# tspooner/rl_markets

Hardware: NVIDIA H100
Metric: env steps/sec (batched LOBs) (higher is better)
Workload: dtype f64

## Files before the change

### rl_markets_b200/csrc/rlm_agent.cuh

```cuda
#pragma once
#include "rlm_env.cuh"

#define FULL 0xffffffffu
#define HS_EMPTY (-1)

__device__ __noinline__ unsigned long long mt_next(unsigned long long* x, int& p) {
  int k = p; if (k >= 312) k -= 312;
  const unsigned long long UM = 0xFFFFFFFF80000000ull, LM = 0x7FFFFFFFull, A = 0xB5026F5AA96619E9ull;
  int k1 = k + 1; if (k1 == 312) k1 = 0;
  int km = k + 156; if (km >= 312) km -= 312;
  unsigned long long y = (__ldcg(x + k) & UM) | (__ldcg(x + k1) & LM);
  unsigned long long z = __ldcg(x + km) ^ (y >> 1) ^ ((y & 1ull) ? A : 0ull);
  __stcg(x + k, z);
  p = k + 1;
  z ^= (z >> 29) & 0x5555555555555555ull;
  z ^= (z << 17) & 0x71D67FFFEDA60000ull;
  z ^= (z << 37) & 0xFFF7EEE000000000ull;
  z ^= z >> 43;
  return z;
}
__device__ __noinline__ double mt_uniform_real(unsigned long long* x, int& p) {
  double r = __ull2double_rn(mt_next(x, p)) / 18446744073709551616.0;
  if (r >= 1.0) r = 0.99999999999999988897769753748;
  return r * (1.0 - 0.0) + 0.0;
// ... 112 lines not shown
    }
    unsigned long long sum = __ldg(rnd + ((lane + 449 * nf) & 2047));
#pragma unroll
    for (int i = 0; i < NF_MAX; ++i) sum += v[i];
    out.s[g] = null_state ? 0ull : sum;
  }
  return out;
}
template <bool POW2>
__device__ __forceinline__ int ln_tile(const LnSums& h, int k) {
  if (POW2) {
    const unsigned lo = (unsigned)h.s[k / RLM_MAX_ACTIONS] + P.rg[k / RLM_MAX_ACTIONS][k % RLM_MAX_ACTIONS];
    return h.null_state ? 0 : (int)(lo & (unsigned)(P.memory_size - 1));
  }
  return h.null_state ? 0 : mod_m(h.s[k / RLM_MAX_ACTIONS] + P.rg[k / RLM_MAX_ACTIONS][k % RLM_MAX_ACTIONS]);
}

#define VROW 33
__device__ __forceinline__ double seg_sum(double acc, double w, const double* r) {
#pragma unroll 8
  for (int i = 0; i < 32; ++i) acc += w * r[i];
  return acc;
}
struct QGather { double a[RLM_MAX_ACTIONS]; double b[RLM_MAX_ACTIONS]; };

__device__ __forceinline__ bool occ_test(const unsigned* occ, int f) { return (__ldcg(occ + (f >> 5)) >> (f & 31)) & 1u; }
__device__ __forceinline__ bool occ_test_s(const unsigned* occ_s, int f) { return (occ_s[f >> 5] >> (f & 31)) & 1u; }

__device__ __forceinline__ void q_issue(const unsigned* rnd, const double* th_a, const double* th_b, const float* vars, int n,
                                        bool null_state, int g, int lane, unsigned long long* bases, bool reuse, int* idx,
// ... 335 lines not shown
```

### rl_markets_b200/csrc/rlm_api.cu

```cuda
#include <cuda_runtime.h>
#include <math.h>
#include <stdio.h>
#include <string.h>
#include <algorithm>
#include <mutex>
#include <string>
#include <vector>

#include "rlm.h"
#include "rlm_flow_tables.h"
#include "rlm_rndseq.h"
#include "rlm_kernels.h"
#include <limits.h>
#include <stddef.h>
#include <stdlib.h>

static thread_local std::string g_err;
static int fail(int code, const std::string& msg) { g_err = msg; return code; }
int rlm_set_error_(int code, const std::string& msg) { return fail(code, msg); }
#define CK(expr)                                                                                      \
  do {                                                                                                \
    cudaError_t _e = (expr);                                                                          \
    if (_e != cudaSuccess) return fail((_e == cudaErrorNoDevice || _e == cudaErrorInsufficientDriver) ? RLM_ERR_NO_DEVICE : RLM_ERR_CUDA, \
                                       std::string(#expr) + ": " + cudaGetErrorString(_e));          \
// ... 314 lines not shown
    CK(cudaMemsetAsync(h->ptr.tape_lo, 0, (size_t)cfg->n_envs * sizeof(int), h->stream));
  }
  g_params_owner = nullptr;
  int rc = upload_params(h);
  if (rc != RLM_OK) return rc;
  CK(rlm_launch_init(h->ptr, cfg->n_envs, 0, h->stream));
  CK(rlm_launch_seed(h->ptr, cfg->n_envs, cfg->random_seed, h->stream));
  if (cfg->random_init) CK(rlm_launch_random_init(h->ptr, h->n_policies, h->stream));
  h->alpha = cfg->alpha_start;
  h->eps = (double)cfg->eps_init;
  h->tau = (double)cfg->tau_init;
  memset(&h->dyn, 0, sizeof(h->dyn));
#ifdef RLM_TIMING
  if (const char* s = getenv("RLM_DEBUG_FLAGS")) h->dyn.debug_flags = atoi(s);
#endif
  if (const char* s = getenv("RLM_ENV_HASH")) h->dyn.env_hash = atoi(s) != 0;
  if (const char* s = getenv("RLM_ROUND_CAP")) h->dyn.round_cap = std::max(0, atoi(s));
  CK(cudaDeviceGetAttribute(&h->n_sms, cudaDevAttrMultiProcessorCount, cfg->device));
  CK(cudaMalloc(&h->ptr.ready, (size_t)cfg->n_envs * 4));
  CK(cudaMalloc(&h->ptr.hsum, (size_t)cfg->n_envs * 3 * 32 * 8));
  h->ready_cap = RLM_READY_CAP;
  CK(cudaMalloc(&h->ptr.ready_count, (size_t)2 * RLM_LIVE_OFF * 4));
  CK(cudaMemset(h->ptr.ready_count, 0, (size_t)2 * RLM_LIVE_OFF * 4));
  CK(cudaMalloc(&h->ptr.runctl, sizeof(RunCtl)));
  CK(cudaMemset(h->ptr.runctl, 0, sizeof(RunCtl)));
  CK(cudaMallocHost(&h->h_live, RLM_MAX_SUB * 2 * sizeof(int)));
  for (int s = 0; s < RLM_MAX_SUB; ++s)
    for (int i = 0; i < 2; ++i) CK(cudaEventCreateWithFlags(&h->ev_live[s][i], cudaEventDisableTiming));
  if (const char* s = getenv("RLM_ROUND_STREAMS")) { const int v = atoi(s); if (v >= 1 && v <= RLM_MAX_SUB) h->round_streams = v; }
  h->n_sub = 1;
  h->staged = !h->hp.is_double && !cfg->shared_policy && cfg->memory_size * 8 <= 65536 && (cfg->memory_size % 2) == 0;
// ... 41 lines not shown
      h->rounds_auto = false;
    }
    if (!getenv("RLM_ROUND_CAP")) h->dyn.round_cap = 3;
    if (const char* s = getenv("RLM_PDL")) rlm_set_pdl(atoi(s));
    if (const char* s = getenv("RLM_AGENT_VARIANT")) { const int v = atoi(s); h->agent_variant = (v == 1 || v == 3) ? v : 4; }
    if (cfg->memory_size > (1LL << 27)) {
      if (h->agent_variant == 4) h->agent_variant = 3;
      if (h->engine == 3) h->engine = 1;
    }
  }
  if (cfg->source == RLM_SOURCE_TAPE) {
    if (h->engine != 1) return fail(RLM_ERR_UNSUPPORTED, "the tape source runs on the tick-synchronous and round-paced engines (RLM_ENGINE=F|f|p read the stream source only)");
    h->dyn.tape_l2 = 1;
    if (const char* s = getenv("RLM_TAPE_PREFETCH")) h->dyn.tape_l2 = atoi(s) != 0;
  }
  cudaDeviceSetLimit(cudaLimitMaxL2FetchGranularity, 32);
  CK(cudaStreamSynchronize(h->stream));
  return RLM_OK;
}

int rlm_destroy(rlm_handle h) {
  API_LOCK;
  if (!h) return RLM_OK;
  cudaSetDevice(h->cfg.device);
  cudaStreamSynchronize(h->stream);
  cudaFree(h->ptr.env); cudaFree(h->ptr.theta); cudaFree(h->ptr.theta_b); cudaFree(h->ptr.dtheta);
  cudaFree(h->ptr.trace_f); cudaFree(h->ptr.trace_e); cudaFree(h->ptr.mt_pol); cudaFree(h->ptr.mt_agt);
  cudaFree(h->ptr.records); cudaFree(h->ptr.record_count); cudaFree(h->ptr.counters);
  cudaFree(h->d_gather); if (h->h_gather) cudaFreeHost(h->h_gather);
  if (h->copy_stream) { cudaStreamSynchronize(h->copy_stream); cudaStreamDestroy(h->copy_stream); }
  for (int i = 0; i < 2; ++i) {
    cudaFree(h->d_stream[i]);
    if (h->ev_copied[i]) cudaEventDestroy(h->ev_copied[i]);
    if (h->ev_consumed[i]) cudaEventDestroy(h->ev_consumed[i]);
  }
  cudaFree(h->ptr.ready); cudaFree(h->ptr.ready_count); cudaFree(h->ptr.occ); cudaFree(h->ptr.hsum);
  cudaFree(h->ptr.runctl); if (h->h_live) cudaFreeHost(h->h_live);
  cudaFree((void*)h->ptr.tape); cudaFree(h->ptr.tape_cur); cudaFree(h->ptr.tape_lo);
  for (auto& es : h->ev_live) for (auto e : es) if (e) cudaEventDestroy(e);
  cudaFree(h->ptr.q_slots); cudaFree(h->ptr.ag_done); cudaFree(h->d_qctl);
  for (auto e : h->ev) cudaEventDestroy(e);
  for (auto& g : h->graphs) cudaGraphExecDestroy(g.exec);
  if (h->ev_fork) cudaEventDestroy(h->ev_fork);
  for (int s = 0; s < RLM_MAX_SUB; ++s) {
    if (h->sub_stream[s]) { cudaStreamSynchronize(h->sub_stream[s]); cudaStreamDestroy(h->sub_stream[s]); }
    if (h->ev_join[s]) cudaEventDestroy(h->ev_join[s]);
  }
  if (h->own_stream && h->stream) cudaStreamDestroy(h->stream);
  if (g_params_owner == h) g_params_owner = nullptr;
  delete h;
  return RLM_OK;
// ... 609 lines not shown
  return RLM_OK;
}
int rlm_write_theta(rlm_handle h, int32_t policy, int32_t table, const double* in, int64_t n) {
  API_LOCK;
  if (!h || !in) return fail(RLM_ERR_INVALID_ARGUMENT, "null argument");
  if (policy < 0 || policy >= h->n_policies || n < 0 || n > h->cfg.memory_size) return fail(RLM_ERR_INVALID_ARGUMENT, "bad policy index / length");
  double* dst = table == 0 ? h->ptr.theta : h->ptr.theta_b;
  if (!dst) return fail(RLM_ERR_INVALID_ARGUMENT, "no such table");
  CK(cudaSetDevice(h->cfg.device));
  CK(cudaStreamSynchronize(h->stream));
  CK(cudaMemcpy(dst + (size_t)policy * h->cfg.memory_size, in, (size_t)n * 8, cudaMemcpyHostToDevice));
  CK(cudaMemset(h->ptr.occ + (size_t)policy * h->hp.occ_words, 0xFF, (size_t)h->hp.occ_words * 4));
  if (!h->cfg.shared_policy) {
    const int dense = (int)h->cfg.memory_size;
    CK(cudaMemcpy(h->ptr.env + (size_t)policy * h->hp.env_stride + offsetof(EnvHdr, ag) + offsetof(AgentD, n_occ), &dense, 4, cudaMemcpyHostToDevice));
  }
  CK(cudaDeviceSynchronize());
  return RLM_OK;
}

int rlm_copy_theta(rlm_handle dst, rlm_handle src) {
  API_LOCK;
  if (!dst || !src) return fail(RLM_ERR_INVALID_ARGUMENT, "null handle");
  if (dst->cfg.device != src->cfg.device || dst->n_policies != src->n_policies || dst->cfg.memory_size != src->cfg.memory_size ||
      dst->hp.is_double != src->hp.is_double || dst->cfg.shared_policy != src->cfg.shared_policy)
    return fail(RLM_ERR_INVALID_ARGUMENT, "rlm_copy_theta: handles differ in device, policy count, memory_size or table count");
  CK(cudaSetDevice(dst->cfg.device));
  CK(cudaStreamSynchronize(src->stream));
  CK(cudaStreamSynchronize(dst->stream));
  const size_t tbytes = (size_t)src->n_policies * (size_t)src->cfg.memory_size * 8;
  CK(cudaMemcpy(dst->ptr.theta, src->ptr.theta, tbytes, cudaMemcpyDeviceToDevice));
  if (src->ptr.theta_b) CK(cudaMemcpy(dst->ptr.theta_b, src->ptr.theta_b, tbytes, cudaMemcpyDeviceToDevice));
  CK(cudaMemcpy(dst->ptr.occ, src->ptr.occ, (size_t)src->n_policies * (size_t)src->hp.occ_words * 4, cudaMemcpyDeviceToDevice));
  if (!src->cfg.shared_policy)
    CK(cudaMemcpy2D(dst->ptr.env + offsetof(EnvHdr, ag) + offsetof(AgentD, n_occ), dst->hp.env_stride,
                    src->ptr.env + offsetof(EnvHdr, ag) + offsetof(AgentD, n_occ), src->hp.env_stride, 4, src->cfg.n_envs,
                    cudaMemcpyDeviceToDevice));
  CK(cudaDeviceSynchronize());
  return RLM_OK;
}

int rlm_read_records(rlm_handle h, int32_t env, rlm_step_record* out, int32_t cap, int32_t* n_out) {
  API_LOCK;
  if (!h || !out || !n_out) return fail(RLM_ERR_INVALID_ARGUMENT, "null argument");
  if (env < 0 || env >= h->hp.record_envs) return fail(RLM_ERR_INVALID_ARGUMENT, "env is not recorded (cfg.record_envs)");
  CK(cudaSetDevice(h->cfg.device));
  CK(cudaStreamSynchronize(h->stream));
  int cnt = 0;
  CK(cudaMemcpy(&cnt, h->ptr.record_count + env, 4, cudaMemcpyDeviceToHost));
  int n = std::min(std::min(cnt, h->hp.record_cap), cap);
  if (n > 0) CK(cudaMemcpy(out, h->ptr.records + (size_t)env * h->hp.record_cap, (size_t)n * sizeof(rlm_step_record), cudaMemcpyDeviceToHost));
  *n_out = n;
// ... 285 lines not shown
```

### rl_markets_b200/csrc/rlm_kernels.cu

```cuda
#include <cuda_runtime.h>
#include <stdint.h>
#define RLM_TABLE_QUAL static __device__ const
#include "rlm_flow_tables.h"
#include "rlm_rndseq.h"
#include "rlm_agent.cuh"
#include <cstdio>
#include "rlm_kernels.h"
#define RLM_ENVT_CARVEOUT_DEFAULT 30
#define RLM_SMEM_CARVEOUT 88

#define SCR_Q 0
#define SCR_SS (SCR_Q + 8 * 2 * RLM_MAX_ACTIONS)
#define SCR_IDX (SCR_SS + 4 * SS_SLOTS)
#define SCR_VBUF (SCR_IDX + 4 * 3 * RLM_MAX_ACTIONS * 32)
#define AG_BYTES ((sizeof(AgentD) + 15) & ~(size_t)15)
size_t rlm_scratch_bytes(int is_double) {
  return ((size_t)SCR_VBUF + (size_t)(is_double ? 2 : 1) * RLM_MAX_ACTIONS * VROW * 8 + 15) & ~(size_t)15;
}
size_t rlm_agent_smem_bytes(int warps_per_cta, int scratch_bytes) {
  return (size_t)warps_per_cta * (AG_BYTES + (size_t)scratch_bytes);
}

#define PDL_PROLOGUE() do { asm volatile("griddepcontrol.launch_dependents;" ::: "memory"); asm volatile("griddepcontrol.wait;" ::: "memory"); } while (0)
static bool g_use_pdl = false;
// ... 452 lines not shown
  e.pnl_step += (double)e.position * mpm;
  e.momentum_pnl_step += (double)e.position * mpm;
  e.agg_r += get_reward(e);
  e.agg_pnl += e.pnl_step;
  e.agg_mpm += mpm;
  if (!is_terminal(e) && fabs(e.agg_mpm) < 1e-5) return -1;
  e.pnl_step = e.agg_pnl;
  window_push(e, ring, W_PNLUP, fmax(0.0, e.pnl_step), oldv[W_PNLUP]);
  window_push(e, ring, W_PNLDN, fabs(fmin(0.0, e.pnl_step)), oldv[W_PNLDN]);
  e.ep_reward += e.agg_r;
  e.ep_bandh += e.agg_mpm;
#pragma unroll 1
  for (int i = 0; i < P.n_state_vars; ++i) e.ag.to_vars[i] = (float)get_variable(e, ring, P.state_vars[i]);
  e.ag.last_reward = get_reward(e);
  e.ag.kind = 0;
  e.ag.hs_valid = 0;
  return 0;
}

template <int THREADS, bool TAPE>
__global__ void __launch_bounds__(THREADS) rlm_env_kernel(DevPtrs ptr, DynParams D, int tslot, int only_begin) {
  const int b = D.env0 + blockIdx.x * THREADS + threadIdx.x;
  const int lane = threadIdx.x & 31;
  if (!only_begin) KLOG_BEGIN(0);
  int ready = -1;
  unsigned ticked = 0, errs = 0;
  bool starved = false;
  if (b < (D.n_sub > 0 ? D.env0 + D.n_sub : P.n_envs)) {
    EnvHdr* g = (EnvHdr*)(ptr.env + (size_t)b * P.env_stride);
    const int2 tc = (TAPE && !only_begin) ? ptr.tape_cur[b] : make_int2(0, 0);
    const int ph = g->phase;
// ... 51 lines not shown
          ready = env_tick(e, ring, msg, D.backtest);
          if (was != PH_PREOPEN && ready != -2) ticked = 1;
          if (ready == -2) ready = -1;
        }
      }
      if (ready >= 0 && !ag_in) {
        const int kind = e.ag.kind;
        const double rew = e.ag.last_reward;
        float tv[RLM_N_STATE_MAX];
        for (int i = 0; i < RLM_N_STATE_MAX; ++i) tv[i] = (i < P.n_state_vars) ? e.ag.to_vars[i] : 0.0f;
        const int4* src = (const int4*)g;
        int4* dst = (int4*)&e;
        for (int i = HOT16; i < ALL16; ++i) dst[i] = src[i];
        e.ag.kind = kind;
        if (kind == 0) {
          e.ag.last_reward = rew; e.ag.hs_valid = 0;
          for (int i = 0; i < RLM_N_STATE_MAX; ++i) if (i < P.n_state_vars) e.ag.to_vars[i] = tv[i];
        }
        ag_in = true;
      }
      errs = (unsigned)(e.err | e.ag.err);
      {
        int4* dst = (int4*)g;
        const int4* src = (const int4*)&e;
        for (int i = 0; i < HOT16; ++i) dst[i] = src[i];
        if (ag_in) for (int i = HOT16; i < ALL16; ++i) dst[i] = src[i];
      }
    }
  }
  if (D.hold) {
    bool still = false;
// ... 157 lines not shown
    __syncwarp();
    ready = *w.flag;
    if (ready == 0) {
      if (lane == W_PNLUP || lane == W_PNLDN) window_push(e, ring, lane, pushv[lane], oldv[lane]);
      __syncwarp();
      {
        const bool has = lane < P.n_state_vars;
        const int var = has ? P.state_vars[lane] : -1;
        double x0 = 0.0, x1 = 0.0;
        const bool two = has && var_tick_args(e, ring, var, x0, x1);
        int t0 = 0, t1 = 0, lerr = 0, hint = e.tk_band;
        if (two) { t0 = to_ticks(x0, &lerr, &hint); t1 = to_ticks(x1, &lerr, &hint); }
        if (lerr) atomicOr(&e.err, lerr);
        if (has) e.ag.to_vars[lane] = (float)(two ? var_from_ticks(var, t0, t1) : get_variable(e, ring, var));
      }
      if (lane == 31) { e.ag.last_reward = get_reward(e); e.ag.kind = 0; }
      if (D.env_hash && !D.backtest && !P.shared_policy && P.algorithm < RLM_ALGO_R_LEARN) {
        __syncwarp();
        const LnSums h = ln_hash(rlm_rndseq_table, e.ag.to_vars, false, lane);
        unsigned long long* hs = ptr.hsum + (size_t)env * 96;
        hs[lane] = h.s[0]; hs[32 + lane] = h.s[1]; hs[64 + lane] = h.s[2];
        const double* th_a = ptr.theta + (size_t)env * (size_t)P.memory_size;
        const double* th_b = ptr.theta_b ? ptr.theta_b + (size_t)env * (size_t)P.memory_size : nullptr;
#pragma unroll 1
        for (int g = 0; g < 3; ++g) {
#pragma unroll
          for (int a = 0; a < RLM_MAX_ACTIONS; ++a) {
            if (a < P.n_actions) {
              const int f = mod_m(h.s[g] + P.rg[g][a]);
              asm volatile("prefetch.global.L2 [%0];" ::"l"(th_a + f));
              if (th_b) asm volatile("prefetch.global.L2 [%0];" ::"l"(th_b + f));
            }
          }
        }
        if (lane == 0) e.ag.hs_valid = 1;
      }
    } else if (ready == 1 && D.backtest) {
      if (lane < P.n_state_vars) e.ag.to_vars[lane] = (float)get_variable(e, ring, P.state_vars[lane]);
    }
  }
  __syncwarp();
  return ready;
}

template <bool TAPE>
__global__ void __launch_bounds__(ENVW_WARPS * 32) rlm_env_kernel_w(DevPtrs ptr, DynParams D, int tslot, int only_begin) {
  PDL_PROLOGUE();
  extern __shared__ __align__(16) unsigned char smem[];
  const int tid = threadIdx.x, lane = tid & 31, warp = tid >> 5;
  const int env = D.env0 + blockIdx.x * (blockDim.x >> 5) + warp;
  if (!only_begin) KLOG_BEGIN(0);
  if (env >= (D.n_sub > 0 ? D.env0 + D.n_sub : P.n_envs)) return;
  const EnvWarp w = envw_carve(smem + (size_t)warp * envw_warp_bytes());
  EnvHdr& e = *w.e;
  EnvHdr* g = (EnvHdr*)(ptr.env + (size_t)env * P.env_stride);
  double* ring = (double*)((unsigned char*)g + sizeof(EnvHdr));
  if (only_begin && !g->ag.need_begin) return;
// ... 14 lines not shown
      starved = tc.x >= tc.y;
      if (!starved) {
        ready = envw_tick<true>(w, ring, ptr, D, env, tc.x, tc.y, lane, ticked, tape_word);
        if (lane == 0) ptr.tape_cur[env].x = tc.x + 1;
      }
    } else if (D.ctl_stream) {
      const int4 rc4 = __ldg((const int4*)ptr.runctl);
      DevPtrs pt = ptr;
      pt.stream = (const rlm_tick_msg*)__ldg((const unsigned long long*)ptr.runctl + 2);
      ready = envw_tick(w, ring, pt, D, env, rc4.z + tslot, rc4.w, lane, ticked);
    } else {
      ready = envw_tick(w, ring, ptr, D, env, D.stream_off + tslot, D.stream_ticks, lane, ticked);
    }
  }
  __syncwarp();
  envw_stage_out(g, &e, lane);
  if (!only_begin) KLOG_END(0);
  if (lane == 0) {
    if (ready >= 0) ptr.ready[atomicAdd(&ptr.ready_count[tslot], 1)] = env;
    if (D.hold && ready < 0 && e.phase != PH_DONE && !starved) atomicAdd(&ptr.counters[5], 1ull);
    if (ticked) atomicAdd(&ptr.counters[0], 1ull);
    const unsigned errs = (unsigned)(e.err | e.ag.err);
    if (errs) atomicOr(&ptr.counters[4], (unsigned long long)errs);
  }
}

template <bool TAPE>
__global__ void __launch_bounds__(ENVW_WARPS * 32, 4) rlm_env_round_kernel(DevPtrs ptr, DynParams D, int tslot) {
  PDL_PROLOGUE();
  extern __shared__ __align__(16) unsigned char smem[];
  const int tid = threadIdx.x, lane = tid & 31, warp = tid >> 5;
// ... 36 lines not shown
      ++tc.x;
    } else {
      ready = envw_tick(w, ring, pt, D, env, rc.stream_off + pos, rc.stream_ticks, lane, ticked);
    }
    ++pos; ++n_run;
    if (ready >= 0) break;
  }
  if (lane == 0) {
    e.run_id = rc.run_id; e.run_pos = pos;
    if (tape) {
      ptr.tape_cur[env].x = tc.x;
      if (D.tape_l2 && tc.x < tc.y) asm volatile("prefetch.global.L2 [%0];" ::"l"(ptr.tape + tc.x));
    }
  }
  __syncwarp();
  envw_stage_out(g, &e, lane);
  KLOG_END(0);
  if (lane == 0) {
    if (ready >= 0) ptr.ready[atomicAdd(&ptr.ready_count[tslot], 1)] = env;
    if (ready >= 0 || (e.phase != PH_DONE && pos < rc.n_ticks && !starved)) atomicAdd(&live_count[tslot], 1);
    if (ticked) atomicAdd(&ptr.counters[0], (unsigned long long)ticked);
    const unsigned errs = (unsigned)(e.err | e.ag.err);
    if (errs) atomicOr(&ptr.counters[4], (unsigned long long)errs);
  }
}
__global__ void rlm_runctl_kernel(RunCtl* dst, RunCtl v) { *dst = v; }

__device__ __forceinline__ void emit_record(const DevPtrs& ptr, const EnvHdr* g, int env, const AgentD& ag, const double* theta_a,
                                         const float* vars, int lane) {
  const int* tf = ptr.trace_f + (size_t)env * P.trace_cap;
  const float* te = ptr.trace_e + (size_t)env * P.trace_cap;
// ... 1085 lines not shown
```

### rl_markets_b200/csrc/rlm_learn.cuh

```cuda
#pragma once

#ifndef LN_WARPS
#define LN_WARPS 3
#endif
#define LN_MIN_CTAS (15 / LN_WARPS)
#ifdef RLM_TIMING
#define LPH(i) do { if (lane == 0 && tp_idx < 4096) g_phase_clk[tp_idx * 16 + (i)] = clock64(); } while (0)
#else
#define LPH(i) do { } while (0)
#endif
#define LN_VROW 98
#define LN_AG_BYTES 704

__host__ __device__ inline size_t ln_v_bytes(int is_double) { return (size_t)(is_double ? 2 : 1) * RLM_MAX_ACTIONS * LN_VROW * 8; }
#ifndef UT_LOG2
#define UT_LOG2 10
#endif
#define UT_SLOTS (1 << UT_LOG2)
#define UT_MAX_ENTRIES (UT_SLOTS / 2)
__host__ __device__ inline size_t ln_scratch_bytes(int is_double) {
  return (ln_v_bytes(is_double) + TT_SLOTS * 4 + 2 * UT_SLOTS * 4 + 8 * 2 * RLM_MAX_ACTIONS + 48 + 15) & ~(size_t)15;
}
__host__ __device__ inline size_t ln_warp_bytes(int is_double) { return (size_t)LN_AG_BYTES + ln_scratch_bytes(is_double); }
static_assert(sizeof(AgentD) <= LN_AG_BYTES, "agent block outgrew its shared-memory slot");

template <int K0, int N>
__device__ __forceinline__ void ln_gather_issue(const double* __restrict__ th, const LnSums& h, double* v) {
  const int A = P.n_actions;
  if (P.m_pow2) {
#pragma unroll
    for (int k = 0; k < N; ++k) v[k] = (((K0 + k) % RLM_MAX_ACTIONS) < A) ? __ldcg(th + ln_tile<true>(h, K0 + k)) : 0.0;
  } else {
#pragma unroll
    for (int k = 0; k < N; ++k) v[k] = (((K0 + k) % RLM_MAX_ACTIONS) < A) ? __ldcg(th + ln_tile<false>(h, K0 + k)) : 0.0;
  }
}
template <int K0, int N>
__device__ __forceinline__ void ln_gather_store(const double* v, int lane, double* V) {
  const int A = P.n_actions;
#pragma unroll
  for (int k = 0; k < N; ++k)
    if (((K0 + k) % RLM_MAX_ACTIONS) < A) V[((K0 + k) % RLM_MAX_ACTIONS) * LN_VROW + ((K0 + k) / RLM_MAX_ACTIONS) * 32 + lane] = v[k];
}
template <bool DBL, int GB>
__device__ __forceinline__ void ln_gather(const double* __restrict__ th_a, const double* __restrict__ th_b, const LnSums& h, int lane, double* V) {
  static_assert(GB == 27 || GB == 9, "gather batch: everything, or one feature group at a time");
  double v[GB];
  if (GB == 27) {
    ln_gather_issue<0, GB>(th_a, h, v); ln_gather_store<0, GB>(v, lane, V);
    if (DBL) { ln_gather_issue<0, GB>(th_b, h, v); ln_gather_store<0, GB>(v, lane, V + RLM_MAX_ACTIONS * LN_VROW); }
  } else {
// ... 129 lines not shown
    slot = (slot + 1) & (TT_SLOTS - 1);
  }
}

__device__ __forceinline__ void ln_tt_build(int* tt, const AgentD& ag, int lane) {
  int4* t4 = (int4*)tt;
#pragma unroll
  for (int i = 0; i < TT_SLOTS / 4 / 32; ++i) t4[lane + 32 * i] = make_int4(HS_EMPTY, HS_EMPTY, HS_EMPTY, HS_EMPTY);
  __syncwarp();
  if (!ag.null_from) {
    const int b0 = ag.from_base0[lane];
#pragma unroll 1
    for (int a = 0; a < P.n_actions; ++a) ptt_insert(tt, tile0_from_base(b0, a), a);
  }
  __syncwarp();
}

__device__ __forceinline__ int ln_trace_pass(AgentD& e, const int* tt, int* ut, bool track, int* tf, float* te, double* theta, int action,
                                          float rate, double scaled_update, int lane, const LnSums& h, double* Vp) {
  const bool null_from = e.null_from != 0;
  const int b0 = e.from_base0[lane];
  const float tol = 0.01f;
  int w = 0;
  int ins = 0;
#define LN_UT_FLUSH() do { __syncwarp(); ln_patch_local_ool(ut, scaled_update, h.s[0], h.s[1], h.s[2], h.null_state, lane, Vp); __syncwarp(); ut_clear(ut, lane); __syncwarp(); ins = 0; } while (0)
  if (rate != 0.0f) {
    const int n = e.n_traces;
#pragma unroll 1
    for (int base = 0; base < n; base += 32 * TR_AHEAD) {
      int fq[TR_AHEAD];
// ... 133 lines not shown
  const bool dbg_nofence = false, dbg_nopatch = false;
#endif
  const int kind = ag.kind;
  const int al = lane & 15;
  const bool do_main = (stage != 2) && (kind == 0);
  const bool do_pre = (stage == 2) ? (kind == 0) : (kind == 1 || (kind == 0 && stage == 1));
  const int n_evals = (do_pre ? 1 : 0) + (do_main ? 1 : 0);
  LnSums h;
  h.s[0] = h.s[1] = h.s[2] = 0ull; h.null_state = true;
  double q = 0.0;
#pragma unroll 1
  for (int ev = 0; ev < n_evals; ++ev) {
    const bool is_main = do_main && (ev == n_evals - 1);
    const float* vars = (is_main || stage == 2) ? ag.to_vars : ag.from_vars;
    const bool null_state = is_main ? false : ((kind == 1 || stage == 1) ? ag.null_from != 0 : false);
    if (is_main && ag.hs_valid) {
      const unsigned long long* hs = ptr.hsum + (size_t)env * 96;
      h.s[0] = __ldcg(hs + lane); h.s[1] = __ldcg(hs + 32 + lane); h.s[2] = __ldcg(hs + 64 + lane);
      h.null_state = false;
    } else {
      h = ln_hash(rnd, vars, null_state, lane);
    }
    LPH(2);
    if (DBL || GB != 27) {
      if (is_main) ln_tt_build(tt, ag, lane);
      ln_gather<DBL, GB>(theta_a, theta_b, h, lane, V);
    } else {
      double v[3 * RLM_MAX_ACTIONS];
      ln_gather_issue<0, 27>(theta_a, h, v);
      LPH(3);
      if (is_main) ln_tt_build(tt, ag, lane);
      LPH(4);
      ln_gather_store<0, 27>(v, lane, V);
    }
    __syncwarp();
    LPH(5);
    q = ln_sums(V, DBL, lane);
    __syncwarp();
    LPH(6);
// ... 26 lines not shown
      __syncwarp();
      rate = (float)dec[0];
      scaled = dec[1];
      table = (DBL && dec[2] != 0.0) ? 1 : 0;
    }
    __syncwarp();
    LPH(7);
    int* tf = ptr.trace_f + (size_t)env * P.trace_cap;
    float* te = ptr.trace_e + (size_t)env * P.trace_cap;
    double* th = table ? theta_b : theta_a;
    if (stage == 1) th = table ? ptr.dtheta + P.memory_size : ptr.dtheta;
    const bool local_patch = (stage == 0) && !dbg_nopatch;
    if (local_patch) { ut_clear(ut, lane); __syncwarp(); }
    const int nz = ln_trace_pass(ag, tt, ut, local_patch, tf, te, th, ag.cur_action, rate, scaled, lane, h,
                                 V + (table ? RLM_MAX_ACTIONS * LN_VROW : 0));
    if (lane == 0) { ag.n_traces = nz; ag.sum_traces += nz; ag.hs_valid = 0; }
    sum_z += (lane == 0) ? (unsigned long long)nz : 0ull;
    __syncwarp();
    LPH(8);
    if (env < P.record_envs && !dbg_nofence) __threadfence();
    LPH(9);
    if (env < P.record_envs) { if (RESIDENT) emit_record_res(ptr, hdr, env, ag, theta_a, ag.to_vars, lane); else emit_record_ool(ptr, g, env, ag, theta_a, ag.to_vars, lane); }
    if (stage == 0) {
      if (lane < RLM_N_STATE_MAX + 3) { ag.prev_vars[lane] = ag.from_vars[lane]; ag.from_vars[lane] = ag.to_vars[lane]; }
      ag.from_base0[lane] = mod_m(h.s[0]);
      if (lane == 0) { ag.prev_null = ag.null_from; ag.null_from = 0; ag.n_steps++; ag.ep_step++; ag.need_begin = 1; }
      steps_done++;
      LPH(13);
      if (local_patch) ln_patch_local(ut, scaled, h.s[0], h.s[1], h.s[2], h.null_state, lane, V + (table ? RLM_MAX_ACTIONS * LN_VROW : 0));
      LPH(14);
      __syncwarp();
// ... 359 lines not shown
      int4 t1 = make_int4(0, 0, 0, 0);
      if (lane + 32 < N16) t1 = __ldcg(src + lane + 32);
      dst[lane] = t0;
      if (lane + 32 < N16) dst[lane + 32] = t1;
    }
    __syncwarp();
    const int kind = ag.kind;
    const bool main_step = kind == 0;
    if (main_step) {
      const int n_tr = ag.n_traces;
      if (lane * 32 < n_tr) {
        asm volatile("prefetch.global.L2 [%0];" ::"l"(ptr.trace_f + (size_t)env * P.trace_cap + lane * 32));
        asm volatile("prefetch.global.L2 [%0];" ::"l"(ptr.trace_e + (size_t)env * P.trace_cap + lane * 32));
      }
    }
    LnSums h;
    const bool null_state = (kind == 1) && ag.null_from != 0;
    if (main_step && ag.hs_valid) {
      const unsigned long long* hs = ptr.hsum + (size_t)env * 96;
      h.s[0] = __ldcg(hs + lane); h.s[1] = __ldcg(hs + 32 + lane); h.s[2] = __ldcg(hs + 64 + lane);
      h.null_state = false;
    } else {
      h = ln_hash(rnd, main_step ? ag.to_vars : ag.from_vars, null_state, lane);
    }
    if (P.m_pow2) {
#pragma unroll
      for (int k = 0; k < 3 * RLM_MAX_ACTIONS; ++k)
        if ((k % RLM_MAX_ACTIONS) < A) idx_s[(k % RLM_MAX_ACTIONS) * LS_IROW + (k / RLM_MAX_ACTIONS) * 32 + lane] = (unsigned short)ln_tile<true>(h, k);
    } else {
#pragma unroll
      for (int k = 0; k < 3 * RLM_MAX_ACTIONS; ++k)
        if ((k % RLM_MAX_ACTIONS) < A) idx_s[(k % RLM_MAX_ACTIONS) * LS_IROW + (k / RLM_MAX_ACTIONS) * 32 + lane] = (unsigned short)ln_tile<false>(h, k);
    }
    if (main_step) ln_tt_build(tt, ag, lane);
    __syncwarp();
    {
      unsigned done = 0;
      while (!done)
        asm volatile("{ .reg .pred p; mbarrier.try_wait.parity.shared::cta.b64 p, [%1], %2; selp.u32 %0, 1, 0, p; }" : "=r"(done) : "r"(mbar_a), "r"(parity) : "memory");
// ... 68 lines not shown
        if (total > P.trace_cap) {
          if (lane == 0) ag.err |= ERR_TRACE_OVERFLOW;
          add = add && (pos < P.trace_cap);
          total = P.trace_cap;
        }
        if (add) {
          __stcg(tf + pos, f);
          __stcg(te + pos, 1.0f);
          const double nv = tab[f] + scaled * (double)1.0f;
          tab[f] = nv;
          __stcg(theta + f, nv);
        }
        w = total;
      }
      __syncwarp();
      if (lane == 0) { ag.n_traces = w; ag.sum_traces += w; ag.hs_valid = 0; }
      sum_z += (lane == 0) ? (unsigned long long)w : 0ull;
      if (env < P.record_envs) { __threadfence(); emit_record_ool(ptr, g, env, ag, theta, ag.to_vars, lane); }
      if (lane < RLM_N_STATE_MAX + 3) { ag.prev_vars[lane] = ag.from_vars[lane]; ag.from_vars[lane] = ag.to_vars[lane]; }
      ag.from_base0[lane] = mod_m(h.s[0]);
      if (lane == 0) { ag.prev_null = ag.null_from; ag.null_from = 0; ag.n_steps++; ag.ep_step++; ag.need_begin = 1; }
      steps_done++;
      __syncwarp();
      q = ls_sums(tab, idx_s, lane);
      if (lane < A) { ag.q_from[lane] = q; ag.qb_from[lane] = 0.0; }
    }
    __syncwarp();
    {
      int4* dst = (int4*)&g->ag;
      const int4* src = (const int4*)&ag;
      __stcg(dst + lane, src[lane]);
// ... 36 lines not shown
```

### rl_markets_b200/csrc/rlm_types.h

```cpp
#pragma once
#include <stdint.h>
#include "rlm.h"

#define RLM_NWIN 10
enum { W_MID = 0, W_VLT, W_VNUM, W_VDEN, W_SPREAD, W_TP, W_ASKTX, W_BIDTX, W_PNLUP, W_PNLDN };

enum { PH_PREOPEN = 0, PH_WARMUP = 1, PH_RUN = 2, PH_DONE = 3 };

enum {
  ERR_BAD_PRICE = 1,
  ERR_TICK_RANGE = 2,
  ERR_TRACE_OVERFLOW = 4,
  ERR_INVALID_STATE = 8,
  ERR_STREAM_UNDERRUN = 16
};

struct OrderD {
  double price;
  long long size, q_head, q_tail, executed, initial_queue;
  int live;
  int transactions;
};

struct SideD {
// ... 18 lines not shown
  float from_vars[RLM_N_STATE_MAX + 3];
  float to_vars[RLM_N_STATE_MAX + 3];
  int from_base0[32];
  int crand_r[31];
  int crand_f, crand_b;
  int mt_pol_idx, mt_agt_idx;
  int null_from;
  int n_traces, cur_action;
  int need_begin;
  int kind;
  int ep_step, err;
  int n_occ;
  double rho;
  float prev_vars[RLM_N_STATE_MAX + 3];
  int prev_null;
  int hs_valid;
  int pad[2];
};

struct FillD { long long volume; double proxy, value; };

struct EnvHdr {
  SideD side[2];
  long long position;
  double pnl_step, momentum_pnl_step, ask_quote, bid_quote;
  double agg_r, agg_pnl, agg_mpm;
  double tp_val, ewma_up, ewma_dn;
  double ep_reward, ep_pnl, ep_bandh;
  double w_sum[RLM_NWIN], w_mean[RLM_NWIN], w_s[RLM_NWIN];
  long long n_ticks;
  int w_head[RLM_NWIN], w_count[RLM_NWIN];
// ... 47 lines not shown
  VenueD venue;
  rlm_flow_params flow;
};

struct DynParams {
  double alpha, eps, tau;
  int greedy;
  int n_ticks;
  int stream_ticks;
  int stream_off;
  int env0;
  int backtest;
  int n_sub;
  int sub_idx;
  int debug_flags;
  int env_hash;
  int round_cap;
  int ctl_stream;
  int hold;
  int tape_l2;
};

#define RLM_MAX_SUB 8
#define RLM_READY_CAP 256
#define RLM_LIVE_OFF (RLM_MAX_SUB * RLM_READY_CAP)

struct RunCtl { int run_id, n_ticks, stream_off, stream_ticks; const rlm_tick_msg* stream; long long pad; };

struct DevPtrs {
  unsigned char* env;
  double* theta;
  double* theta_b;
  double* dtheta;
  int* trace_f;
  float* trace_e;
  unsigned long long* mt_pol;
  unsigned long long* mt_agt;
  const rlm_tick_msg* stream;
  rlm_step_record* records;
  int* record_count;
  unsigned long long* counters;
  unsigned* occ;
  unsigned long long* hsum;
  int* ready;
  int* ready_count;
  int* q_slots;
  unsigned* q_head;
  unsigned* q_tail;
  unsigned* env_warps_done;
  int* q_done;
  int* ag_done;
  int q_size;
  int pad;
  RunCtl* runctl;
  const rlm_tick_msg* tape;
  int2* tape_cur;
  int* tape_lo;
};
// ... 1 lines not shown
```

Baseline: 12.30 million.

## Pre-gather next-state theta rows in env kernel for async agent copy

Replaces the opt-in env-side hash and L2 prefetch with a default-on pregather. The env warp now computes the tile hash and gathers the theta values for every tiling and action into a per-env global row buffer. The agent kernel then pulls those rows into shared memory with cp.async, overlapping the copy with the trace-table build. This takes the dependent random gathers off the agent's critical path. The cost is extra global writes and reads plus a new per-env buffer, and the rows could go stale if theta changes between the gather and its use.

```diff
diff --git a/rl_markets_b200/csrc/rlm_agent.cuh b/rl_markets_b200/csrc/rlm_agent.cuh
--- a/rl_markets_b200/csrc/rlm_agent.cuh
+++ b/rl_markets_b200/csrc/rlm_agent.cuh
@@ -150,6 +150,18 @@
     return h.null_state ? 0 : (int)(lo & (unsigned)(P.memory_size - 1));
   }
   return h.null_state ? 0 : mod_m(h.s[k / RLM_MAX_ACTIONS] + P.rg[k / RLM_MAX_ACTIONS][k % RLM_MAX_ACTIONS]);
+}
+
+template <int K0, int N>
+__device__ __forceinline__ void ln_gather_issue(const double* __restrict__ th, const LnSums& h, double* v) {
+  const int A = P.n_actions;
+  if (P.m_pow2) {
+#pragma unroll
+    for (int k = 0; k < N; ++k) v[k] = (((K0 + k) % RLM_MAX_ACTIONS) < A) ? __ldcg(th + ln_tile<true>(h, K0 + k)) : 0.0;
+  } else {
+#pragma unroll
+    for (int k = 0; k < N; ++k) v[k] = (((K0 + k) % RLM_MAX_ACTIONS) < A) ? __ldcg(th + ln_tile<false>(h, K0 + k)) : 0.0;
+  }
 }
 
 #define VROW 33
diff --git a/rl_markets_b200/csrc/rlm_api.cu b/rl_markets_b200/csrc/rlm_api.cu
--- a/rl_markets_b200/csrc/rlm_api.cu
+++ b/rl_markets_b200/csrc/rlm_api.cu
@@ -352,7 +352,6 @@
 #ifdef RLM_TIMING
   if (const char* s = getenv("RLM_DEBUG_FLAGS")) h->dyn.debug_flags = atoi(s);
 #endif
-  if (const char* s = getenv("RLM_ENV_HASH")) h->dyn.env_hash = atoi(s) != 0;
   if (const char* s = getenv("RLM_ROUND_CAP")) h->dyn.round_cap = std::max(0, atoi(s));
   CK(cudaDeviceGetAttribute(&h->n_sms, cudaDevAttrMultiProcessorCount, cfg->device));
   CK(cudaMalloc(&h->ptr.ready, (size_t)cfg->n_envs * 4));
@@ -424,6 +423,9 @@
     h->dyn.tape_l2 = 1;
     if (const char* s = getenv("RLM_TAPE_PREFETCH")) h->dyn.tape_l2 = atoi(s) != 0;
   }
+  h->dyn.pregather = !cfg->shared_policy && cfg->algorithm < RLM_ALGO_R_LEARN && h->agent_variant == 4 && !h->staged &&
+                     h->engine == 1 && h->env_variant == 0;
+  if (h->dyn.pregather) CK(cudaMalloc(&h->ptr.vrow, (size_t)cfg->n_envs * (p.is_double ? 2 : 1) * RLM_MAX_ACTIONS * RLM_PG_ROW * 8));
   cudaDeviceSetLimit(cudaLimitMaxL2FetchGranularity, 32);
   CK(cudaStreamSynchronize(h->stream));
   return RLM_OK;
@@ -444,7 +446,7 @@
     if (h->ev_copied[i]) cudaEventDestroy(h->ev_copied[i]);
     if (h->ev_consumed[i]) cudaEventDestroy(h->ev_consumed[i]);
   }
-  cudaFree(h->ptr.ready); cudaFree(h->ptr.ready_count); cudaFree(h->ptr.occ); cudaFree(h->ptr.hsum);
+  cudaFree(h->ptr.ready); cudaFree(h->ptr.ready_count); cudaFree(h->ptr.occ); cudaFree(h->ptr.hsum); cudaFree(h->ptr.vrow);
   cudaFree(h->ptr.runctl); if (h->h_live) cudaFreeHost(h->h_live);
   cudaFree((void*)h->ptr.tape); cudaFree(h->ptr.tape_cur); cudaFree(h->ptr.tape_lo);
   for (auto& es : h->ev_live) for (auto e : es) if (e) cudaEventDestroy(e);
@@ -1084,6 +1086,7 @@
   if (!h->cfg.shared_policy) {
     const int dense = (int)h->cfg.memory_size;
     CK(cudaMemcpy(h->ptr.env + (size_t)policy * h->hp.env_stride + offsetof(EnvHdr, ag) + offsetof(AgentD, n_occ), &dense, 4, cudaMemcpyHostToDevice));
+    CK(cudaMemset(h->ptr.env + (size_t)policy * h->hp.env_stride + offsetof(EnvHdr, ag) + offsetof(AgentD, pg_valid), 0, 4));
   }
   CK(cudaDeviceSynchronize());
   return RLM_OK;
@@ -1106,6 +1109,7 @@
     CK(cudaMemcpy2D(dst->ptr.env + offsetof(EnvHdr, ag) + offsetof(AgentD, n_occ), dst->hp.env_stride,
                     src->ptr.env + offsetof(EnvHdr, ag) + offsetof(AgentD, n_occ), src->hp.env_stride, 4, src->cfg.n_envs,
                     cudaMemcpyDeviceToDevice));
+  CK(cudaMemset2D(dst->ptr.env + offsetof(EnvHdr, ag) + offsetof(AgentD, pg_valid), dst->hp.env_stride, 0, 4, dst->cfg.n_envs));
   CK(cudaDeviceSynchronize());
   return RLM_OK;
 }
diff --git a/rl_markets_b200/csrc/rlm_kernels.cu b/rl_markets_b200/csrc/rlm_kernels.cu
--- a/rl_markets_b200/csrc/rlm_kernels.cu
+++ b/rl_markets_b200/csrc/rlm_kernels.cu
@@ -490,7 +490,7 @@
   for (int i = 0; i < P.n_state_vars; ++i) e.ag.to_vars[i] = (float)get_variable(e, ring, P.state_vars[i]);
   e.ag.last_reward = get_reward(e);
   e.ag.kind = 0;
-  e.ag.hs_valid = 0;
+  e.ag.pg_valid = 0;
   return 0;
 }
 
@@ -572,7 +572,7 @@
         for (int i = HOT16; i < ALL16; ++i) dst[i] = src[i];
         e.ag.kind = kind;
         if (kind == 0) {
-          e.ag.last_reward = rew; e.ag.hs_valid = 0;
+          e.ag.last_reward = rew; e.ag.pg_valid = 0;
           for (int i = 0; i < RLM_N_STATE_MAX; ++i) if (i < P.n_state_vars) e.ag.to_vars[i] = tv[i];
         }
         ag_in = true;
@@ -760,33 +760,42 @@
         if (lerr) atomicOr(&e.err, lerr);
         if (has) e.ag.to_vars[lane] = (float)(two ? var_from_ticks(var, t0, t1) : get_variable(e, ring, var));
       }
-      if (lane == 31) { e.ag.last_reward = get_reward(e); e.ag.kind = 0; }
-      if (D.env_hash && !D.backtest && !P.shared_policy && P.algorithm < RLM_ALGO_R_LEARN) {
-        __syncwarp();
-        const LnSums h = ln_hash(rlm_rndseq_table, e.ag.to_vars, false, lane);
-        unsigned long long* hs = ptr.hsum + (size_t)env * 96;
-        hs[lane] = h.s[0]; hs[32 + lane] = h.s[1]; hs[64 + lane] = h.s[2];
-        const double* th_a = ptr.theta + (size_t)env * (size_t)P.memory_size;
-        const double* th_b = ptr.theta_b ? ptr.theta_b + (size_t)env * (size_t)P.memory_size : nullptr;
-#pragma unroll 1
-        for (int g = 0; g < 3; ++g) {
-#pragma unroll
-          for (int a = 0; a < RLM_MAX_ACTIONS; ++a) {
-            if (a < P.n_actions) {
-              const int f = mod_m(h.s[g] + P.rg[g][a]);
-              asm volatile("prefetch.global.L2 [%0];" ::"l"(th_a + f));
-              if (th_b) asm volatile("prefetch.global.L2 [%0];" ::"l"(th_b + f));
-            }
-          }
-        }
-        if (lane == 0) e.ag.hs_valid = 1;
-      }
+      const bool pg = D.pregather && !D.backtest;
+      if (lane == 31) { e.ag.last_reward = get_reward(e); e.ag.kind = 0; e.ag.pg_valid = pg ? 1 : 0; }
     } else if (ready == 1 && D.backtest) {
       if (lane < P.n_state_vars) e.ag.to_vars[lane] = (float)get_variable(e, ring, P.state_vars[lane]);
     }
   }
   __syncwarp();
   return ready;
+}
+
+__device__ __forceinline__ void pg_store(const double* v, double* vr) {
+#pragma unroll
+  for (int a = 0; a < RLM_MAX_ACTIONS; ++a)
+    if (a < P.n_actions) __stcg(vr + a * RLM_PG_ROW, v[a]);
+}
+template <int K0>
+__device__ __forceinline__ void pg_group(const double* th, const LnSums& h, double* vr) {
+  double v[RLM_MAX_ACTIONS];
+  ln_gather_issue<K0, RLM_MAX_ACTIONS>(th, h, v);
+  pg_store(v, vr + (K0 / RLM_MAX_ACTIONS) * 32);
+}
+__device__ __forceinline__ double* pg_gather(const DevPtrs& ptr, int env, const float* to_vars, int lane, double* v) {
+  const LnSums h = ln_hash(rlm_rndseq_table, to_vars, false, lane);
+  unsigned long long* hs = ptr.hsum + (size_t)env * 96;
+  hs[lane] = h.s[0]; hs[32 + lane] = h.s[1]; hs[64 + lane] = h.s[2];
+  const size_t tab = (size_t)RLM_MAX_ACTIONS * RLM_PG_ROW;
+  double* vr = ptr.vrow + (size_t)env * (P.is_double ? 2 : 1) * tab + lane;
+  const double* th = ptr.theta + (size_t)env * (size_t)P.memory_size;
+  if (P.is_double) {
+    pg_group<0>(th, h, vr); pg_group<9>(th, h, vr); pg_group<18>(th, h, vr);
+    th = ptr.theta_b + (size_t)env * (size_t)P.memory_size;
+    vr += tab;
+  }
+  pg_group<0>(th, h, vr); pg_group<9>(th, h, vr);
+  ln_gather_issue<18, RLM_MAX_ACTIONS>(th, h, v);
+  return vr + 64;
 }
 
 template <bool TAPE>
@@ -831,7 +840,11 @@
     }
   }
   __syncwarp();
+  const bool pg = ready == 0 && D.pregather && !D.backtest;
+  double pv[RLM_MAX_ACTIONS];
+  double* pvr = pg ? pg_gather(ptr, env, e.ag.to_vars, lane, pv) : nullptr;
   envw_stage_out(g, &e, lane);
+  if (pg) pg_store(pv, pvr);
   if (!only_begin) KLOG_END(0);
   if (lane == 0) {
     if (ready >= 0) ptr.ready[atomicAdd(&ptr.ready_count[tslot], 1)] = env;
@@ -898,7 +911,11 @@
     }
   }
   __syncwarp();
+  const bool pg = ready == 0 && D.pregather && !D.backtest;
+  double pv[RLM_MAX_ACTIONS];
+  double* pvr = pg ? pg_gather(ptr, env, e.ag.to_vars, lane, pv) : nullptr;
   envw_stage_out(g, &e, lane);
+  if (pg) pg_store(pv, pvr);
   KLOG_END(0);
   if (lane == 0) {
     if (ready >= 0) ptr.ready[atomicAdd(&ptr.ready_count[tslot], 1)] = env;
diff --git a/rl_markets_b200/csrc/rlm_learn.cuh b/rl_markets_b200/csrc/rlm_learn.cuh
--- a/rl_markets_b200/csrc/rlm_learn.cuh
+++ b/rl_markets_b200/csrc/rlm_learn.cuh
@@ -24,17 +24,6 @@
 __host__ __device__ inline size_t ln_warp_bytes(int is_double) { return (size_t)LN_AG_BYTES + ln_scratch_bytes(is_double); }
 static_assert(sizeof(AgentD) <= LN_AG_BYTES, "agent block outgrew its shared-memory slot");
 
-template <int K0, int N>
-__device__ __forceinline__ void ln_gather_issue(const double* __restrict__ th, const LnSums& h, double* v) {
-  const int A = P.n_actions;
-  if (P.m_pow2) {
-#pragma unroll
-    for (int k = 0; k < N; ++k) v[k] = (((K0 + k) % RLM_MAX_ACTIONS) < A) ? __ldcg(th + ln_tile<true>(h, K0 + k)) : 0.0;
-  } else {
-#pragma unroll
-    for (int k = 0; k < N; ++k) v[k] = (((K0 + k) % RLM_MAX_ACTIONS) < A) ? __ldcg(th + ln_tile<false>(h, K0 + k)) : 0.0;
-  }
-}
 template <int K0, int N>
 __device__ __forceinline__ void ln_gather_store(const double* v, int lane, double* V) {
   const int A = P.n_actions;
@@ -194,6 +183,29 @@
     for (int a = 0; a < P.n_actions; ++a) ptt_insert(tt, tile0_from_base(b0, a), a);
   }
   __syncwarp();
+}
+
+template <bool DBL>
+__device__ __forceinline__ void ln_rows_issue(const double* __restrict__ vr, int lane, double* V) {
+  constexpr int ROW = RLM_PG_ROW / 2;
+  constexpr int TOTAL = (DBL ? 2 : 1) * RLM_MAX_ACTIONS * ROW;
+  const int A = P.n_actions;
+  const double2* src = (const double2*)vr;
+  const unsigned vs = (unsigned)__cvta_generic_to_shared(V);
+#pragma unroll
+  for (int i = 0; i < (TOTAL + 31) / 32; ++i) {
+    const int k = lane + 32 * i, row = k / ROW;
+    if (k < TOTAL && row % RLM_MAX_ACTIONS < A)
+      asm volatile("cp.async.cg.shared.global [%0], [%1], 16;" ::"r"(vs + (unsigned)(row * LN_VROW + 2 * (k % ROW)) * 8), "l"(src + k) : "memory");
+  }
+  asm volatile("cp.async.commit_group;" ::: "memory");
+}
+template <bool DBL>
+__device__ __noinline__ void ln_rows_copy(const double* vr, const AgentD& ag, int* tt, int lane, double* V) {
+  ASSUME_SHARED(&ag); ASSUME_SHARED(tt); ASSUME_SHARED(V);
+  ln_rows_issue<DBL>(vr, lane, V);
+  ln_tt_build(tt, ag, lane);
+  asm volatile("cp.async.wait_group 0;" ::: "memory");
 }
 
 __device__ __forceinline__ int ln_trace_pass(AgentD& e, const int* tt, int* ut, bool track, int* tf, float* te, double* theta, int action,
@@ -357,7 +369,8 @@
     const bool is_main = do_main && (ev == n_evals - 1);
     const float* vars = (is_main || stage == 2) ? ag.to_vars : ag.from_vars;
     const bool null_state = is_main ? false : ((kind == 1 || stage == 1) ? ag.null_from != 0 : false);
-    if (is_main && ag.hs_valid) {
+    const bool pre = !RESIDENT && is_main && ag.pg_valid;
+    if (pre) {
       const unsigned long long* hs = ptr.hsum + (size_t)env * 96;
       h.s[0] = __ldcg(hs + lane); h.s[1] = __ldcg(hs + 32 + lane); h.s[2] = __ldcg(hs + 64 + lane);
       h.null_state = false;
@@ -365,7 +378,9 @@
       h = ln_hash(rnd, vars, null_state, lane);
     }
     LPH(2);
-    if (DBL || GB != 27) {
+    if (pre) {
+      ln_rows_copy<DBL>(ptr.vrow + (size_t)env * (DBL ? 2 : 1) * (RLM_MAX_ACTIONS * RLM_PG_ROW), ag, tt, lane, V);
+    } else if (DBL || GB != 27) {
       if (is_main) ln_tt_build(tt, ag, lane);
       ln_gather<DBL, GB>(theta_a, theta_b, h, lane, V);
     } else {
@@ -422,7 +437,7 @@
     if (local_patch) { ut_clear(ut, lane); __syncwarp(); }
     const int nz = ln_trace_pass(ag, tt, ut, local_patch, tf, te, th, ag.cur_action, rate, scaled, lane, h,
                                  V + (table ? RLM_MAX_ACTIONS * LN_VROW : 0));
-    if (lane == 0) { ag.n_traces = nz; ag.sum_traces += nz; ag.hs_valid = 0; }
+    if (lane == 0) { ag.n_traces = nz; ag.sum_traces += nz; ag.pg_valid = 0; }
     sum_z += (lane == 0) ? (unsigned long long)nz : 0ull;
     __syncwarp();
     LPH(8);
@@ -812,15 +827,8 @@
         asm volatile("prefetch.global.L2 [%0];" ::"l"(ptr.trace_e + (size_t)env * P.trace_cap + lane * 32));
       }
     }
-    LnSums h;
     const bool null_state = (kind == 1) && ag.null_from != 0;
-    if (main_step && ag.hs_valid) {
-      const unsigned long long* hs = ptr.hsum + (size_t)env * 96;
-      h.s[0] = __ldcg(hs + lane); h.s[1] = __ldcg(hs + 32 + lane); h.s[2] = __ldcg(hs + 64 + lane);
-      h.null_state = false;
-    } else {
-      h = ln_hash(rnd, main_step ? ag.to_vars : ag.from_vars, null_state, lane);
-    }
+    const LnSums h = ln_hash(rnd, main_step ? ag.to_vars : ag.from_vars, null_state, lane);
     if (P.m_pow2) {
 #pragma unroll
       for (int k = 0; k < 3 * RLM_MAX_ACTIONS; ++k)
@@ -919,7 +927,7 @@
         w = total;
       }
       __syncwarp();
-      if (lane == 0) { ag.n_traces = w; ag.sum_traces += w; ag.hs_valid = 0; }
+      if (lane == 0) { ag.n_traces = w; ag.sum_traces += w; }
       sum_z += (lane == 0) ? (unsigned long long)w : 0ull;
       if (env < P.record_envs) { __threadfence(); emit_record_ool(ptr, g, env, ag, theta, ag.to_vars, lane); }
       if (lane < RLM_N_STATE_MAX + 3) { ag.prev_vars[lane] = ag.from_vars[lane]; ag.from_vars[lane] = ag.to_vars[lane]; }
diff --git a/rl_markets_b200/csrc/rlm_types.h b/rl_markets_b200/csrc/rlm_types.h
--- a/rl_markets_b200/csrc/rlm_types.h
+++ b/rl_markets_b200/csrc/rlm_types.h
@@ -3,6 +3,7 @@
 #include "rlm.h"
 
 #define RLM_NWIN 10
+#define RLM_PG_ROW 96
 enum { W_MID = 0, W_VLT, W_VNUM, W_VDEN, W_SPREAD, W_TP, W_ASKTX, W_BIDTX, W_PNLUP, W_PNLDN };
 
 enum { PH_PREOPEN = 0, PH_WARMUP = 1, PH_RUN = 2, PH_DONE = 3 };
@@ -56,7 +57,7 @@
   double rho;
   float prev_vars[RLM_N_STATE_MAX + 3];
   int prev_null;
-  int hs_valid;
+  int pg_valid;
   int pad[2];
 };
 
@@ -134,7 +135,7 @@
   int n_sub;
   int sub_idx;
   int debug_flags;
-  int env_hash;
+  int pregather;
   int round_cap;
   int ctl_stream;
   int hold;
@@ -162,6 +163,7 @@
   unsigned long long* counters;
   unsigned* occ;
   unsigned long long* hsum;
+  double* vrow;
   int* ready;
   int* ready_count;
   int* q_slots;
```

After: 13.10 million (median of 6 runs). 6.5% higher.
